# plumk97/pip

Hardware: AMD Instinct MI355X
Metric: GiB/s payload checksummed (device-resident), MTU-9000 TCP batch; Mpkt/s (higher is better)
Workload: dtype u8

## Files before the change

### pip_amd/csrc/pipck_coop.hip

```cpp
#include "pipck_common.hpp"
#include "pipck_device.hpp"

#include <algorithm>

namespace pipck {

constexpr uint32_t kCoopLoadsOnly = 1u << 21;
constexpr uint32_t kCoopNoEnd = 1u << 22;

template <int U>
constexpr int coop_waves_per_simd() { return U >= 32 ? 2 : (U >= 24 ? 3 : (U >= 16 ? 4 : 5)); }

__host__ __device__ constexpr uint32_t coop_pitch(uint32_t k) { return k | 1u; }

template <int U, bool VERIFY, bool NT, bool PROBE>
__device__ __forceinline__ void coop_body(uint32_t* s_part, const uint8_t* __restrict__ arena, uint32_t cpp,
                                          uint32_t len, uint64_t n, uint32_t K, const uint32_t* __restrict__ pseudo,
                                          uint32_t n_flows, const uint32_t* __restrict__ flow_of, uint64_t flow_origin,
                                          uint16_t* __restrict__ out, uint8_t* __restrict__ ok, uint32_t kflags,
                                          uint32_t* __restrict__ err) {
    if (!PROBE) kflags &= ~(kCoopLoadsOnly | kCoopNoEnd);
    const int lane = threadIdx.x & 63;
    const uint32_t w = (uint32_t)__builtin_amdgcn_readfirstlane((int)(threadIdx.x >> 6));
    const uint32_t pitch = coop_pitch(K);
    const uint64_t p0 = (uint64_t)blockIdx.x * K;
    const uint32_t np = (uint32_t)min<uint64_t>((uint64_t)K, n - p0);
    const uint32_t tchunks = np * cpp;
    const uint32_t rows = (tchunks + 63) >> 6;
    const uint32_t nch = (len + 15) >> 4;
    const int tail = nch ? (int)len - 16 * ((int)nch - 1) : 16;
    for (uint32_t i = threadIdx.x; i < 64u * pitch; i += 256) s_part[i] = 0;
    uint32_t Pb = 0;
    bool fbad = false;
    if (pseudo && threadIdx.x < np) {
        const uint64_t pkt = p0 + threadIdx.x;
        Pb = flow_of ? flow_pseudo(pseudo, flow_of[pkt], n_flows, fbad)
                     : pseudo[(uint32_t)((flow_origin + pkt) % n_flows)];
    }
    __syncthreads();
    const buf_t tb = buf_rsrc(reinterpret_cast<const u32x4*>(arena) + p0 * cpp, tchunks * 16u);
    uint32_t* part = s_part + lane * pitch;
    const uint32_t q = 256u / cpp, rm = 256u % cpp;
    uint32_t pkt = (64u * w) / cpp, k0 = (64u * w) % cpp;
    const uint32_t my_rows = rows > w ? (rows - w + 3) >> 2 : 0u;
    u32x4 v[U];
    uint32_t probe = 0;
#pragma unroll
    for (int u = 0; u < U; u++) v[u] = buf_load<NT>(tb, ((w + 4u * u) * 64u + lane) * 16u);
    for (uint32_t j0 = 0; j0 < my_rows; j0 += U) {
#pragma unroll
        for (int u = 0; u < U; u++) {
            const uint32_t j = j0 + u;
            if (j < my_rows && (kflags & kCoopLoadsOnly)) {
                probe += v[u].x;
            } else if (j < my_rows) {
                uint32_t k = k0 + lane, pk = pkt;
                if (k >= cpp) {
                    k -= cpp;
                    pk++;
                }
                u32x4 x = v[u];
                if (k >= nch) x = u32x4{0u, 0u, 0u, 0u};
                else if (k == nch - 1 && tail < 16) x = mask_tail(x, tail);
                if (pk < np) atomicAdd(&part[pk], dot4(x, 0u));
                k0 += rm;
                pkt += q;
                if (k0 >= cpp) {
                    k0 -= cpp;
                    pkt++;
                }
            }
            v[u] = buf_load<NT>(tb, ((w + 4u * (j + U)) * 64u + lane) * 16u);
        }
    }
    __syncthreads();
    if (kflags & (kCoopLoadsOnly | kCoopNoEnd)) {
        if (probe == 0x9E3779B9u) s_part[0] = probe;
        return;
    }
    const uint32_t i = threadIdx.x;
    if (i < np) {
        uint32_t s = 0;
#pragma unroll 16
        for (int l = 0; l < 64; l++) s += s_part[l * pitch + i];
        const uint32_t F = bswap16(fold16(s));
        const uint32_t P = pseudo ? Pb + len_term(len) : 0u;
        if (fbad) flow_refused(err);
        if (VERIFY)
            store_result8(buf_rsrc(ok + p0, np), i, fbad ? 0u : (uint32_t)(fold16(P + F) == 0xFFFFu));
        else
            store_result16(buf_rsrc(out + p0, 2u * np), 2u * i, fbad ? 0u : (uint32_t)finish(P, F));
    }
}

template <int U, bool VERIFY, bool NT>
__global__ __launch_bounds__(256) __attribute__((amdgpu_waves_per_eu(coop_waves_per_simd<U>()))) void k_flat_coop(
    const uint8_t* __restrict__ arena, uint32_t cpp, uint32_t len, uint64_t n, uint32_t K,
    const uint32_t* __restrict__ pseudo, uint32_t n_flows, const uint32_t* __restrict__ flow_of, uint64_t flow_origin,
    uint16_t* __restrict__ out, uint8_t* __restrict__ ok, uint32_t kflags, uint32_t* __restrict__ err) {
    extern __shared__ uint32_t s_part[];
    coop_body<U, VERIFY, NT, false>(s_part, arena, cpp, len, n, K, pseudo, n_flows, flow_of, flow_origin, out, ok,
                                    kflags, err);
}

template <int U, bool VERIFY, bool NT>
__global__ __launch_bounds__(256) __attribute__((amdgpu_waves_per_eu(coop_waves_per_simd<U>()))) void
k_flat_coop_probe(const uint8_t* __restrict__ arena, uint32_t cpp, uint32_t len, uint64_t n, uint32_t K,
                  const uint32_t* __restrict__ pseudo, uint32_t n_flows, const uint32_t* __restrict__ flow_of,
                  uint64_t flow_origin, uint16_t* __restrict__ out, uint8_t* __restrict__ ok, uint32_t kflags,
                  uint32_t* __restrict__ err) {
    extern __shared__ uint32_t s_part[];
    coop_body<U, VERIFY, NT, true>(s_part, arena, cpp, len, n, K, pseudo, n_flows, flow_of, flow_origin, out, ok,
                                   kflags, err);
}

typedef void (*coop_fn)(const uint8_t*, uint32_t, uint32_t, uint64_t, uint32_t, const uint32_t*, uint32_t,
                        const uint32_t*, uint64_t, uint16_t*, uint8_t*, uint32_t, uint32_t*);

int launch_flat_coop(bool verify, const void* d_arena, uint64_t stride, uint32_t len, uint64_t n,
                     const uint32_t* d_pseudo, uint32_t n_flows, const uint32_t* d_flow_of, uint64_t flow_origin,
                     uint16_t* d_out, uint8_t* d_ok, uint32_t* d_err, hipStream_t s, uint32_t rows_per_wave,
                     uint32_t ring, uint32_t kflags) {
    const uint32_t cpp = (uint32_t)(stride / 16);
    const bool jumbo = cpp >= 256;
    const uint32_t rpw = rows_per_wave ? rows_per_wave : (jumbo ? 64u : 48u);
    uint32_t K = (4u * rpw * 64u) / cpp;
    K = std::max<uint32_t>(8u, std::min<uint32_t>(256u, K / 8u * 8u));
    if ((uint64_t)K * cpp * 16u >= (1ull << 31)) return PIPCK_EINVAL;
    const uint64_t blocks = (n + K - 1) / K;
    if (blocks > 0x7FFFFFFFull) return PIPCK_EINVAL;
    const size_t lds = 64u * coop_pitch(K) * sizeof(uint32_t);
    const uint32_t nf = n_flows ? n_flows : 1u;
    const uint32_t u = ring ? ring : 32u;
    static const coop_fn kCoop[3][2] = {
        {k_flat_coop<16, false, true>, k_flat_coop<16, true, true>},
        {k_flat_coop<24, false, true>, k_flat_coop<24, true, true>},
        {k_flat_coop<32, false, true>, k_flat_coop<32, true, true>}};
    static const coop_fn kCoopProbe[3] = {k_flat_coop_probe<16, false, true>, k_flat_coop_probe<24, false, true>,
                                          k_flat_coop_probe<32, false, true>};
    const int ui = u >= 32 ? 2 : (u >= 24 ? 1 : 0);
    const bool probe = (kflags & (kCoopLoadsOnly | kCoopNoEnd)) && !verify;
    PIPCK_LAUNCH(probe ? kCoopProbe[ui] : kCoop[ui][verify], dim3((uint32_t)blocks), dim3(256), lds, s, (const uint8_t*)d_arena, cpp, len, n,
                 K, d_pseudo, nf, d_flow_of, flow_origin, d_out, d_ok, kflags, d_err);
    PIPCK_LAUNCHED("k_flat_coop");
    return PIPCK_OK;
}

}
```

### pip_amd/engine.py

```python
from __future__ import annotations

import ctypes as C

from . import _lib
from ._lib import Desc, Flow4, Flow6, call, check, load

DESC_BYTES = C.sizeof(Desc)


def _torch():
    import torch

    return torch


def _ptr(t) -> C.c_void_p | None:
    return None if t is None else C.c_void_p(t.data_ptr())


def current_stream(device=None) -> C.c_void_p:
    torch = _torch()
    return C.c_void_p(torch.cuda.current_stream(device).cuda_stream)


def require_gpu() -> None:
    torch = _torch()
    if not torch.cuda.is_available():
        raise RuntimeError("pip_amd engine needs a HIP device (gfx950); none is visible")
    load()


_hip = None


def hip_runtime() -> C.CDLL:
    global _hip
    if _hip is None:
        import os

        load()
        paths = set()
        with open("/proc/self/maps") as f:
            for line in f:
                parts = line.split()
                if len(parts) >= 6 and os.path.basename(parts[5]).startswith("libamdhip64.so"):
                    paths.add(os.path.realpath(parts[5]))
        if len(paths) != 1:
            raise RuntimeError(f"expected exactly one HIP runtime mapped in this process, found {sorted(paths)}")
        _hip = C.CDLL(paths.pop(), mode=os.RTLD_NOLOAD | os.RTLD_GLOBAL)
    return _hip


def pci_bus_id(device: int) -> str:
    buf = C.create_string_buffer(64)
    try:
        if hip_runtime().hipDeviceGetPCIBusId(buf, C.c_int(len(buf)), C.c_int(device)) == 0:
            return buf.value.decode()
    except (OSError, RuntimeError):
        pass
    p = _torch().cuda.get_device_properties(device)
    return f"{getattr(p, 'pci_domain_id', 0):04x}:{getattr(p, 'pci_bus_id', 0):02x}:" \
           f"{getattr(p, 'pci_device_id', 0):02x}.0"


def gen_flows(family: int, n_flows: int, seed: int, proto: int, device=None):
    torch = _torch()
    size = C.sizeof(Flow4 if family == 4 else Flow6)
    flows = torch.empty(n_flows * size, dtype=torch.uint8, device=device or "cuda")
    fn = "pipck_gen_flows4" if family == 4 else "pipck_gen_flows6"
    call(fn, _ptr(flows), n_flows, seed, proto, current_stream(flows.device))
    return flows, prepare_flows(family, flows, n_flows)


def prepare_flows(family: int, flows, n_flows: int):
    torch = _torch()
    pseudo = torch.empty(n_flows, dtype=torch.int32, device=flows.device)
    fn = "pipck_flows4_prepare" if family == 4 else "pipck_flows6_prepare"
    call(fn, _ptr(flows), n_flows, _ptr(pseudo), current_stream(flows.device))
    return pseudo


def flows_to_device(family: int, flows_bytes: bytes, device=None):
    torch = _torch()
    t = torch.frombuffer(bytearray(flows_bytes), dtype=torch.uint8).to(device or "cuda")
    return t


def _n_flows(n_flows, pseudo, flow_of) -> int:
    if n_flows is not None:
        return n_flows
    if flow_of is not None and pseudo is not None:
        return pseudo.numel()
    return 1


def checksum_fixed(arena, stride: int, length: int, n: int, pseudo=None, n_flows: int | None = None, flow_of=None,
                   flow_origin: int = 0, out=None, err=None):
    torch = _torch()
    if out is None:
        out = torch.empty(n, dtype=torch.int16, device=arena.device)
    _check_span(arena, stride, length, n)
    call("pipck_checksum_fixed_n", _ptr(arena), stride, length, n, _ptr(pseudo), _n_flows(n_flows, pseudo, flow_of),
         _ptr(flow_of), flow_origin, _ptr(out), _ptr(err), current_stream(arena.device))
    return out


def _bound(fn: str, *args):
    f = getattr(load(), fn)

    def run():
        rc = f(*args)
        if rc:
            check(fn, rc)

    return run


def prepare_checksum_fixed(arena, stride: int, length: int, n: int, pseudo=None, n_flows: int | None = None,
                           flow_of=None, flow_origin: int = 0, out=None, err=None):
    torch = _torch()
    if out is None:
        out = torch.empty(n, dtype=torch.int16, device=arena.device)
    _check_span(arena, stride, length, n)
    return _bound("pipck_checksum_fixed_n", _ptr(arena), stride, length, n, _ptr(pseudo),
                  _n_flows(n_flows, pseudo, flow_of), _ptr(flow_of), flow_origin, _ptr(out), _ptr(err),
                  current_stream(arena.device)), out


def verify_fixed(arena, stride: int, length: int, n: int, pseudo=None, n_flows: int | None = None, flow_of=None,
                 flow_origin: int = 0, ok=None, err=None):
    torch = _torch()
    if ok is None:
        ok = torch.empty(n, dtype=torch.uint8, device=arena.device)
    _check_span(arena, stride, length, n)
    call("pipck_verify_fixed_n", _ptr(arena), stride, length, n, _ptr(pseudo), _n_flows(n_flows, pseudo, flow_of),
         _ptr(flow_of), flow_origin, _ptr(ok), _ptr(err), current_stream(arena.device))
    return ok


def checksum_ragged(arena, desc, pseudo=None, out=None, err=None):
    torch = _torch()
    n = desc.shape[0]
    if out is None:
        out = torch.empty(n, dtype=torch.int16, device=arena.device)
    call("pipck_checksum_ragged_n", _ptr(arena), _nbytes(arena), _ptr(desc), n, _ptr(pseudo),
         pseudo.numel() if pseudo is not None else 0, _ptr(out), _ptr(err), current_stream(arena.device))
    return out


def verify_ragged(arena, desc, pseudo=None, ok=None, err=None):
    torch = _torch()
    n = desc.shape[0]
    if ok is None:
        ok = torch.empty(n, dtype=torch.uint8, device=arena.device)
    call("pipck_verify_ragged_n", _ptr(arena), _nbytes(arena), _ptr(desc), n, _ptr(pseudo),
         pseudo.numel() if pseudo is not None else 0, _ptr(ok), _ptr(err), current_stream(arena.device))
    return ok


def tune_xcd_weights(m=None, period: int = 0) -> None:
    arr = (C.c_uint32 * 8)(*[int(x) for x in m]) if m is not None else None
    call("pipck_tune_xcd_weights", arr, period)


def _nbytes(t) -> int:
    return t.numel() * t.element_size()


def checksum_packed(arena, lens, tile_chunk, n: int | None = None, pseudo=None, n_flows: int | None = None,
                    flow_of=None, flow_origin: int = 0, out=None, err=None):
    torch = _torch()
    n = lens.numel() if n is None else n
    if out is None:
        out = torch.empty(n, dtype=torch.int16, device=arena.device)
    _check_packed(arena, lens, tile_chunk, n)
    call("pipck_checksum_packed_n", _ptr(arena), _nbytes(arena), _ptr(lens), _ptr(tile_chunk), n, _ptr(pseudo),
         _n_flows(n_flows, pseudo, flow_of), _ptr(flow_of), flow_origin, _ptr(out), _ptr(err),
         current_stream(arena.device))
    return out


def verify_packed(arena, lens, tile_chunk, n: int | None = None, pseudo=None, n_flows: int | None = None,
                  flow_of=None, flow_origin: int = 0, ok=None, err=None):
    torch = _torch()
    n = lens.numel() if n is None else n
    if ok is None:
        ok = torch.empty(n, dtype=torch.uint8, device=arena.device)
    _check_packed(arena, lens, tile_chunk, n)
    call("pipck_verify_packed_n", _ptr(arena), _nbytes(arena), _ptr(lens), _ptr(tile_chunk), n, _ptr(pseudo),
         _n_flows(n_flows, pseudo, flow_of), _ptr(flow_of), flow_origin, _ptr(ok), _ptr(err),
         current_stream(arena.device))
    return ok


def packed_index(lens, n: int | None = None):
    torch = _torch()
    n = lens.numel() if n is None else n
    tc = torch.empty((n + 63) // 64 + 1, dtype=torch.int64, device=lens.device)
    call("pipck_packed_index", _ptr(lens), n, _ptr(tc), current_stream(lens.device))
    return tc


_packed_total: dict = {}


def _check_packed(arena, lens, tile_chunk, n, unit: int = 16):
    import weakref

    if n > lens.numel() or tile_chunk.numel() < (n + 63) // 64 + 1:
        raise ValueError("lens / tile_chunk shorter than the batch")
    ent = _packed_total.get(id(tile_chunk))
    if ent is not None and ent[0]() is tile_chunk and ent[1] == tile_chunk._version and ent[2] == n:
        chunks = ent[3]
    else:
        chunks = int(tile_chunk[(n + 63) // 64].item())
        if len(_packed_total) > 64:
            _packed_total.clear()
        _packed_total[id(tile_chunk)] = (weakref.ref(tile_chunk), tile_chunk._version, n, chunks)
    need = unit * chunks if unit == 16 else (chunks + 15) // 16 * 16
    if need > arena.numel() * arena.element_size():
        raise ValueError(f"packed batch needs {need} B, arena has {arena.numel() * arena.element_size()}")


def checksum_packed_bytes(arena, lens, tile_off, n: int | None = None, pseudo=None, n_flows: int | None = None,
                          flow_of=None, flow_origin: int = 0, out=None, err=None):
    torch = _torch()
    n = lens.numel() if n is None else n
    if out is None:
        out = torch.empty(n, dtype=torch.int16, device=arena.device)
    _check_packed(arena, lens, tile_off, n, unit=1)
    call("pipck_checksum_packed_bytes_n", _ptr(arena), _nbytes(arena), _ptr(lens), _ptr(tile_off), n, _ptr(pseudo),
         _n_flows(n_flows, pseudo, flow_of), _ptr(flow_of), flow_origin, _ptr(out), _ptr(err),
         current_stream(arena.device))
    return out


def prepare_checksum_packed_bytes(arena, lens, tile_off, n: int | None = None, pseudo=None,
                                  n_flows: int | None = None, flow_of=None, flow_origin: int = 0, out=None, err=None):
    torch = _torch()
    n = lens.numel() if n is None else n
    if out is None:
        out = torch.empty(n, dtype=torch.int16, device=arena.device)
    _check_packed(arena, lens, tile_off, n, unit=1)
    return _bound("pipck_checksum_packed_bytes_n", _ptr(arena), _nbytes(arena), _ptr(lens), _ptr(tile_off), n,
                  _ptr(pseudo), _n_flows(n_flows, pseudo, flow_of), _ptr(flow_of), flow_origin, _ptr(out),
                  _ptr(err), current_stream(arena.device)), out


def verify_packed_bytes(arena, lens, tile_off, n: int | None = None, pseudo=None, n_flows: int | None = None,
                        flow_of=None, flow_origin: int = 0, ok=None, err=None):
    torch = _torch()
    n = lens.numel() if n is None else n
    if ok is None:
        ok = torch.empty(n, dtype=torch.uint8, device=arena.device)
    _check_packed(arena, lens, tile_off, n, unit=1)
    call("pipck_verify_packed_bytes_n", _ptr(arena), _nbytes(arena), _ptr(lens), _ptr(tile_off), n, _ptr(pseudo),
         _n_flows(n_flows, pseudo, flow_of), _ptr(flow_of), flow_origin, _ptr(ok), _ptr(err),
         current_stream(arena.device))
    return ok


def rx_verify_ring(ring, stride: int, lens, n: int | None = None, ok=None, err=None):
    torch = _torch()
    n = lens.numel() if n is None else n
    if n * stride > _nbytes(ring) or n > lens.numel():
        raise ValueError("ring smaller than n * stride, or fewer lengths than slots")
    if ok is None:
        ok = torch.empty(n, dtype=torch.uint8, device=ring.device)
    call("pipck_rx_verify_ring_n", _ptr(ring), stride, _ptr(lens), n, _ptr(ok), _ptr(err),
         current_stream(ring.device))
    return ok


def rx_verify_device(arena, lens, tile_off, n: int | None = None, ok=None, err=None):
    torch = _torch()
    n = lens.numel() if n is None else n
    if ok is None:
        ok = torch.empty(n, dtype=torch.uint8, device=arena.device)
    _check_packed(arena, lens, tile_off, n, unit=1)
    call("pipck_rx_verify_device", _ptr(arena), _nbytes(arena), _ptr(lens), _ptr(tile_off), n, _ptr(ok), _ptr(err),
         current_stream(arena.device))
    return ok


TX_IP_FILLED, TX_L4_FILLED = 1, 2
TX_UDP_ZERO_AS_ONES = 1


def tx_fill_device(arena, lens, tile_off, n: int | None = None, flags: int = 0, done=None, err=None):
    torch = _torch()
    n = lens.numel() if n is None else n
    if done is None:
        done = torch.empty(n, dtype=torch.uint8, device=arena.device)
    _check_packed(arena, lens, tile_off, n, unit=1)
    call("pipck_tx_fill_device", _ptr(arena), _nbytes(arena), _ptr(lens), _ptr(tile_off), n, flags, _ptr(done),
         _ptr(err), current_stream(arena.device))
    return done


def packed_bytes_index(lens, n: int | None = None):
    torch = _torch()
    n = lens.numel() if n is None else n
    to = torch.empty((n + 63) // 64 + 1, dtype=torch.int64, device=lens.device)
    call("pipck_packed_bytes_index", _ptr(lens), n, _ptr(to), current_stream(lens.device))
    return to


def checksum_chains(arena, segs, seg_begin, pkt_flow=None, pseudo=None, out=None, err=None):
    torch = _torch()
    n_pk = seg_begin.shape[0] - 1
    scratch = torch.empty(max(segs.shape[0], 1), dtype=torch.int32, device=arena.device)
    if out is None:
        out = torch.empty(n_pk, dtype=torch.int16, device=arena.device)
    call("pipck_checksum_chains_n", _ptr(arena), _nbytes(arena), _ptr(segs), segs.shape[0], _ptr(seg_begin),
         _ptr(pkt_flow), n_pk, _ptr(pseudo), pseudo.numel() if pseudo is not None else 0, _ptr(scratch), _ptr(out),
         _ptr(err), current_stream(arena.device))
    return out


def update_fixed(arena, stride: int, n: int, cover_off: int, cover_len: int, ck_off: int, edit_off: int,
                 edit_len: int, new_bytes=None, new_stride: int = 0, pseudo_old=None, pseudo_new=None,
                 n_flows: int | None = None, flow_of=None, flow_origin: int = 0, err=None) -> None:
    if pseudo_old is not None and pseudo_new is not None and pseudo_old.numel() != pseudo_new.numel():
        raise ValueError("pseudo_old and pseudo_new must have the same number of flows")
    _check_span(arena, stride, cover_off + cover_len, n)
    if edit_len and new_bytes is not None and n and \
            (n - 1) * new_stride + edit_len > new_bytes.numel() * new_bytes.element_size():
        raise ValueError("new_bytes is too small for the batch")
    call("pipck_update_fixed_n", _ptr(arena), stride, n, cover_off, cover_len, ck_off, edit_off, edit_len,
         _ptr(new_bytes), new_stride, _ptr(pseudo_old), _ptr(pseudo_new), _n_flows(n_flows, pseudo_old, flow_of),
         _ptr(flow_of), flow_origin, _ptr(err), current_stream(arena.device))


def _check_span(arena, stride, length, n):
    if n and (n - 1) * stride + length > arena.numel() * arena.element_size():
        raise ValueError(f"arena of {arena.numel() * arena.element_size()} B is too small for "
                         f"{n} packets x stride {stride} (len {length})")


def make_desc(offsets, lengths, flows, device=None):
    import numpy as np

    torch = _torch()
    n = len(offsets)
    raw = np.zeros(n, dtype=[("offset", "<u8"), ("len", "<u4"), ("flow", "<u4")])
    raw["offset"], raw["len"], raw["flow"] = offsets, lengths, flows
    return torch.from_numpy(raw.view(np.int64).reshape(n, 2).copy()).to(device or "cuda")


def cfg_seed(cfg: int) -> int:
    return load().pipck_cfg_seed(cfg)


def gen_fixed(arena, stride: int, length: int, n: int, first: int, seed: int, hdr: int) -> None:
    _check_span(arena, stride, length, n)
    if n and (n * stride) > arena.numel() * arena.element_size():
        raise ValueError("arena too small for generated stride slots")
    call("pipck_gen_fixed", _ptr(arena), stride, length, n, first, seed, hdr, current_stream(arena.device))


def gen_ragged(n: int, first: int, seed: int, hdr: int, n_flows: int, device=None, lengths=None):
    torch = _torch()
    dev = device or "cuda"
    if lengths is None:
        lengths = torch.empty(n, dtype=torch.int32, device=dev)
        call("pipck_gen_zipf_lengths", _ptr(lengths), n, first, seed, current_stream(lengths.device))
    desc = torch.empty((n, 2), dtype=torch.int64, device=lengths.device)
    nbytes = C.c_uint64(0)
    call("pipck_gen_ragged_layout", _ptr(lengths), n, first, n_flows, _ptr(desc), C.byref(nbytes),
         current_stream(lengths.device))
    arena = torch.empty(max(int(nbytes.value), 16), dtype=torch.uint8, device=lengths.device)
    call("pipck_gen_ragged_fill", _ptr(arena), _ptr(desc), n, first, seed, hdr, current_stream(arena.device))
    return arena, desc, lengths


def gen_packed(n: int, first: int, seed: int, hdr: int, device=None, lengths=None):
    torch = _torch()
    arena, desc, lengths = gen_ragged(n, first, seed, hdr, 1, device=device, lengths=lengths)
    del desc
    lens16 = lengths.to(torch.int16)
    return arena, lens16, packed_index(lens16, n), lengths


def gen_packed_bytes(n: int, first: int, seed: int, hdr: int, device=None, lengths=None):
    torch = _torch()
    dev = device or "cuda"
    if lengths is None:
        lengths = torch.empty(n, dtype=torch.int32, device=dev)
        call("pipck_gen_zipf_lengths", _ptr(lengths), n, first, seed, current_stream(lengths.device))
    lens16 = lengths.to(torch.int16)
    tile_off = packed_bytes_index(lens16, n)
    total = int(tile_off[(n + 63) // 64].item())
    arena = torch.empty(max((total + 15) // 16 * 16, 16), dtype=torch.uint8, device=lengths.device)
    arena[total:].zero_()
    call("pipck_gen_packed_bytes", _ptr(arena), _ptr(lens16), _ptr(tile_off), n, first, seed, hdr,
         current_stream(arena.device))
    return arena, lens16, tile_off, lengths


def gen_rx_ring(n: int, seed: int, stride: int, l4_len: int = 0):
    torch = _torch()
    arena, lens, _, kind, start, l4 = gen_rx_frames(n, seed, l4_len=l4_len)
    ln = lens.to(torch.int64) & 0xFFFF
    if int(ln.max().item()) > stride:
        raise ValueError("a frame is longer than the slot stride")
    ring = torch.zeros(n * stride, dtype=torch.uint8, device=arena.device)
    step = 1 << 16
    for f0 in range(0, n, step):
        lc, sc = ln[f0:f0 + step], start[f0:f0 + step]
        m = lc.numel()
        frame = torch.repeat_interleave(torch.arange(m, device=arena.device), lc)
        excl = torch.cumsum(lc, 0) - lc
        within = torch.arange(frame.numel(), device=arena.device) - excl[frame]
        ring[(f0 + frame) * stride + within] = arena[sc[frame] + within]
    return ring, lens, kind


def gen_rx_frames(n: int, seed: int, checksummed: bool = True, l4_len: int = 0):
    torch = _torch()
    g = torch.Generator(device="cuda").manual_seed(seed)
    l4 = torch.empty(n, dtype=torch.int32, device="cuda")
    if l4_len:
        l4.fill_(l4_len)
    else:
        call("pipck_gen_zipf_lengths", _ptr(l4), n, 0, cfg_seed(4), current_stream())
    kind = torch.randint(0, 4, (n,), device="cuda", generator=g)
    v6 = kind == 3
    hl = torch.where(v6, 40, 20).to(torch.int64)
    l4 = l4.to(torch.int64)
    frame = l4 + hl
    lens = frame.to(torch.int16)
    tile_off = packed_bytes_index(lens)
    total = int(tile_off[-1].item())
    arena = torch.randint(0, 256, ((total + 16 + 127) // 128 * 128,), dtype=torch.uint8, device="cuda", generator=g)
    start = torch.cumsum(frame, 0) - frame
    proto = torch.where(kind == 2, 17, 6)

    def put(col, val, mask):
        idx = (start + col)[mask]
        arena[idx] = (val[mask] if torch.is_tensor(val) else torch.full_like(idx, val)).to(torch.uint8)

    v4 = ~v6
    put(0, 0x45, v4)
    put(2, frame >> 8, v4)
    put(3, frame & 0xFF, v4)
    put(6, 0, v4)
    put(7, 0, v4)
    put(9, proto, v4)
    put(0, 0x60, v6)
    put(4, l4 >> 8, v6)
    put(5, l4 & 0xFF, v6)
    put(6, 6, v6)
    if not checksummed:
        return arena, lens, tile_off, kind, start, l4
    field = start + hl + torch.where(proto == 6, 16, 6)
    for k in (0, 1):
        arena[field + k] = 0
    put(10, 0, v4)
    put(11, 0, v4)

    def be_words(first, count):
        idx = start[:, None] + first + torch.arange(2 * count, device="cuda")
        b = arena[idx].to(torch.int64)
        return (b[:, 0::2] * 256 + b[:, 1::2]).sum(1)

    pseudo = torch.where(v6, be_words(8, 16), be_words(12, 4)) + proto
    flows = torch.arange(n, device="cuda", dtype=torch.int64)

    def ragged(off, ln, ps):
        desc = torch.stack([off, ln | (flows << 32)], 1)
        return checksum_ragged(arena, desc, ps).to(torch.int64) & 0xFFFF

    r = ragged(start + hl, l4, pseudo.to(torch.int32))
    arena[field] = (r >> 8).to(torch.uint8)
    arena[field + 1] = (r & 0xFF).to(torch.uint8)
    ip = ragged(start, torch.full_like(l4, 20), None)
    put(10, ip >> 8, v4)
    put(11, ip & 0xFF, v4)
    return arena, lens, tile_off, kind, start, l4


def tune(lanes_per_packet: int = 0, loads_per_lane: int = 0, blocks: int = 0, plain_loads: bool = False,
         flat: bool = True, nt_loads: bool = False, rows_per_task: int = 0, xcd_groups: bool = False,
         packed_tiles: bool = True, wide_blocks: bool = False,
         small: bool = True, small_k_log: int = 0, flat_small: bool = True, tiny_tiles: bool = True,
         flat_tiny: bool = True, force_flat_tiny: bool = False, packed_marks_only: bool = False,
         trace: bool = False, loads_only: bool = False, no_task_end: bool = False,
         end_no_store: bool = False, alt_flat_schedule: bool = False,
         plain_result_stores: bool = False, wave_stores: bool = False, free_run: bool = False,
         packed_no_align: bool = False, hdr_in_place: bool = False, ring_own_slots: bool = False,
         ring_all_coop: bool = False, ring_adapt: bool | None = None) -> None:
    if not 0 <= small_k_log <= 4:
        raise ValueError("small_k_log must be 0..4")
    flags = ((1 if plain_loads else 0) | (0 if flat else 2) | (4 if nt_loads else 0) | (8 if xcd_groups else 0)
             | (0 if packed_tiles else 16) | (32 if wide_blocks else 0) | (0 if small else 64)
             | (0 if flat_small else 128) | (rows_per_task << 8) | (0 if tiny_tiles else 1 << 16)
             | (0 if flat_tiny else 1 << 17) | (1 << 18 if force_flat_tiny else 0) | (small_k_log << 24)
             | (1 << 19 if packed_marks_only else 0) | (1 << 20 if trace else 0) | (1 << 21 if loads_only else 0) | (1 << 22 if no_task_end else 0)
             | (1 << 23 if end_no_store else 0) | (1 << 28 if alt_flat_schedule else 0)
             | (1 << 29 if plain_result_stores else 0)
             | (1 << 30 if (wave_stores or packed_no_align) else 0)
             | (1 << 31 if free_run else 0))
    load().pipck_tune(lanes_per_packet, loads_per_lane, blocks, flags)
    load().pipck_tune_probes(1 if hdr_in_place else 0)
    ring = (1 if ring_own_slots else 0) | (2 if ring_all_coop else 0) | {None: 0, False: 4, True: 8}[ring_adapt]
    if ring or hasattr(load(), "pipck_tune_ring"):
        load().pipck_tune_ring(ring)
```

Before: 6740.

## Add fixed-depth jumbo cooperative body, line-aligned task sizing, and relax U32 occupancy

Adds an opt-in jumbo-packet body for the cooperative checksum kernel. When a task's chunks fit in two ring passes, it uses a fully unrolled two-stage load/reduce schedule with branchless tail masking, explicit waitcnt and sched barriers, replacing the generic per-row loop and its bookkeeping. Adds an opt-in task sizing rule that rounds packets-per-block to a cache-line-aligned quantum, and a flag for exact waits. It also raises the occupancy hint for the U=32 kernel from 2 to 3 waves per SIMD, which applies by default and may cause register spills in exchange for more latency hiding.

Result: no change. 6759 (median of 2 runs) (+0.3%).

```diff
diff --git a/pip_amd/csrc/pipck_coop.hip b/pip_amd/csrc/pipck_coop.hip
--- a/pip_amd/csrc/pipck_coop.hip
+++ b/pip_amd/csrc/pipck_coop.hip
@@ -9,7 +9,7 @@
 constexpr uint32_t kCoopNoEnd = 1u << 22;
 
 template <int U>
-constexpr int coop_waves_per_simd() { return U >= 32 ? 2 : (U >= 24 ? 3 : (U >= 16 ? 4 : 5)); }
+constexpr int coop_waves_per_simd() { return U >= 24 ? 3 : (U >= 16 ? 4 : 5); }
 
 __host__ __device__ constexpr uint32_t coop_pitch(uint32_t k) { return k | 1u; }
 
@@ -93,14 +93,117 @@
     }
 }
 
+constexpr uint32_t kCoopLineTasks = 1u << 29;
+constexpr uint32_t kCoopJumboBody = 1u << 30;
+constexpr uint32_t kCoopExactWait = 1u << 31;
+
+__host__ __device__ constexpr bool coop_jumbo_fits(uint32_t cpp, uint32_t K, uint32_t U) {
+    return cpp >= 256u && (uint64_t)K * cpp <= 4ull * 64u * 2u * U;
+}
+
+template <int U, bool NT, bool MASK, bool EXACT>
+__device__ __forceinline__ void coop_rows_jumbo(uint32_t* part, buf_t tb, uint32_t w, int lane, uint32_t cpp,
+                                                uint32_t len, uint32_t np) {
+    asm volatile("; coop_rows_jumbo mask=%0 exact=%1" ::"n"((int)MASK), "n"((int)EXACT) : "memory");
+    const uint32_t nch = (len + 15) >> 4;
+    const Mask128 tm = low_bytes(nch ? (int)len - 16 * ((int)nch - 1) : 0);
+    const uint32_t t0 = (uint32_t)tm.m0, t1 = (uint32_t)(tm.m0 >> 32), t2 = (uint32_t)tm.m1,
+                   t3 = (uint32_t)(tm.m1 >> 32);
+    uint32_t k = 64u * w + (uint32_t)lane, pk = 0;
+    const uint32_t off = k * 16u;
+    auto row = [&](u32x4 x) {
+        uint32_t s;
+        if (MASK) {
+            const bool whole = k + 1u < nch;
+            x.x &= whole ? ~0u : t0;
+            x.y &= whole ? ~0u : t1;
+            x.z &= whole ? ~0u : t2;
+            x.w &= whole ? ~0u : t3;
+            const uint32_t d = dot4(x, 0u);
+            s = k < nch ? d : 0u;
+        } else {
+            s = dot4(x, 0u);
+        }
+        atomicAdd(&part[min(pk, np - 1u)], s);
+        const uint32_t t = k + 256u;
+        pk += t >= cpp ? 1u : 0u;
+        k = min(t, t - cpp);
+        __builtin_amdgcn_sched_barrier(0);
+    };
+    u32x4 v[U];
+#pragma unroll
+    for (int u = 0; u < U; u++) v[u] = buf_load<NT>(tb, off + 4096u * u);
+    if (!EXACT) __builtin_amdgcn_s_waitcnt(0x0F70);
+#pragma unroll
+    for (int u = 0; u < U; u++) {
+        row(v[u]);
+        v[u] = buf_load<NT>(tb, off + 4096u * (U + u));
+    }
+    if (!EXACT) __builtin_amdgcn_s_waitcnt(0x0F70);
+#pragma unroll
+    for (int u = 0; u < U; u++) row(v[u]);
+}
+
+template <int U, bool VERIFY, bool NT>
+__device__ __forceinline__ void coop_body_jumbo(uint32_t* s_part, const uint8_t* __restrict__ arena, uint32_t cpp,
+                                                uint32_t len, uint64_t n, uint32_t K,
+                                                const uint32_t* __restrict__ pseudo, uint32_t n_flows,
+                                                const uint32_t* __restrict__ flow_of, uint64_t flow_origin,
+                                                uint16_t* __restrict__ out, uint8_t* __restrict__ ok, uint32_t kflags,
+                                                uint32_t* __restrict__ err) {
+    const int lane = threadIdx.x & 63;
+    const uint32_t w = (uint32_t)__builtin_amdgcn_readfirstlane((int)(threadIdx.x >> 6));
+    const uint32_t pitch = coop_pitch(K);
+    const uint64_t p0 = (uint64_t)blockIdx.x * K;
+    const uint32_t np = (uint32_t)min<uint64_t>((uint64_t)K, n - p0);
+    const uint32_t tchunks = np * cpp;
+    for (uint32_t i = threadIdx.x; i < 64u * pitch; i += 256) s_part[i] = 0;
+    uint32_t Pb = 0;
+    bool fbad = false;
+    if (pseudo && threadIdx.x < np) {
+        const uint64_t pkt = p0 + threadIdx.x;
+        Pb = flow_of ? flow_pseudo(pseudo, flow_of[pkt], n_flows, fbad)
+                     : pseudo[(uint32_t)((flow_origin + pkt) % n_flows)];
+    }
+    __syncthreads();
+    const buf_t tb = buf_rsrc(reinterpret_cast<const u32x4*>(arena) + p0 * cpp, tchunks * 16u);
+    uint32_t* part = s_part + lane * pitch;
+    const bool exact = (kflags & kCoopExactWait) != 0;
+    if (len == cpp * 16u) {
+        if (exact) coop_rows_jumbo<U, NT, false, true>(part, tb, w, lane, cpp, len, np);
+        else coop_rows_jumbo<U, NT, false, false>(part, tb, w, lane, cpp, len, np);
+    } else {
+        if (exact) coop_rows_jumbo<U, NT, true, true>(part, tb, w, lane, cpp, len, np);
+        else coop_rows_jumbo<U, NT, true, false>(part, tb, w, lane, cpp, len, np);
+    }
+    __syncthreads();
+    const uint32_t i = threadIdx.x;
+    if (i < np) {
+        uint32_t s = 0;
+#pragma unroll 16
+        for (int l = 0; l < 64; l++) s += s_part[l * pitch + i];
+        const uint32_t F = bswap16(fold16(s));
+        const uint32_t P = pseudo ? Pb + len_term(len) : 0u;
+        if (fbad) flow_refused(err);
+        if (VERIFY)
+            store_result8(buf_rsrc(ok + p0, np), i, fbad ? 0u : (uint32_t)(fold16(P + F) == 0xFFFFu));
+        else
+            store_result16(buf_rsrc(out + p0, 2u * np), 2u * i, fbad ? 0u : (uint32_t)finish(P, F));
+    }
+}
+
 template <int U, bool VERIFY, bool NT>
 __global__ __launch_bounds__(256) __attribute__((amdgpu_waves_per_eu(coop_waves_per_simd<U>()))) void k_flat_coop(
     const uint8_t* __restrict__ arena, uint32_t cpp, uint32_t len, uint64_t n, uint32_t K,
     const uint32_t* __restrict__ pseudo, uint32_t n_flows, const uint32_t* __restrict__ flow_of, uint64_t flow_origin,
     uint16_t* __restrict__ out, uint8_t* __restrict__ ok, uint32_t kflags, uint32_t* __restrict__ err) {
     extern __shared__ uint32_t s_part[];
-    coop_body<U, VERIFY, NT, false>(s_part, arena, cpp, len, n, K, pseudo, n_flows, flow_of, flow_origin, out, ok,
-                                    kflags, err);
+    if ((kflags & kCoopJumboBody) && coop_jumbo_fits(cpp, K, U))
+        coop_body_jumbo<U, VERIFY, NT>(s_part, arena, cpp, len, n, K, pseudo, n_flows, flow_of, flow_origin, out, ok,
+                                       kflags, err);
+    else
+        coop_body<U, VERIFY, NT, false>(s_part, arena, cpp, len, n, K, pseudo, n_flows, flow_of, flow_origin, out,
+                                        ok, kflags, err);
 }
 
 template <int U, bool VERIFY, bool NT>
@@ -117,15 +220,28 @@
 typedef void (*coop_fn)(const uint8_t*, uint32_t, uint32_t, uint64_t, uint32_t, const uint32_t*, uint32_t,
                         const uint32_t*, uint64_t, uint16_t*, uint8_t*, uint32_t, uint32_t*);
 
+constexpr uint32_t coop_gcd(uint32_t a, uint32_t b) { return b ? coop_gcd(b, a % b) : a; }
+constexpr uint32_t coop_task_packets(uint64_t stride, uint32_t rows_per_wave, bool line_quantum) {
+    const uint32_t cpp = (uint32_t)(stride / 16);
+    const bool jumbo = cpp >= 256;
+    const uint32_t rpw = rows_per_wave ? rows_per_wave : (jumbo ? 64u : 48u);
+    const uint32_t q = jumbo && line_quantum ? 128u / coop_gcd((uint32_t)(stride % 128u), 128u) : 8u;
+    const uint32_t K = (4u * rpw * 64u) / cpp / q * q;
+    return K < q ? q : (K > 256u ? 256u : K);
+}
+static_assert(coop_task_packets(8992, 0, true) == 28 && coop_task_packets(8960, 0, true) == 29, "cfg5 / cfg3, by line");
+static_assert(coop_task_packets(4096, 0, true) == 64 && coop_task_packets(65536, 0, true) == 4, "jumbo, by line");
+static_assert(coop_task_packets(8992, 54, true) == 24, "rows_per_task = 54: cfg5's default task under the line rule");
+static_assert(coop_task_packets(1488, 0, true) == 128 && coop_task_packets(1488, 0, false) == 128, "cfg2");
+static_assert(coop_task_packets(8992, 0, false) == 24 && coop_task_packets(8960, 0, false) == 24, "cfg5 / cfg3");
+static_assert(coop_task_packets(4096, 0, false) == 64 && coop_task_packets(65536, 0, false) == 8, "jumbo");
+
 int launch_flat_coop(bool verify, const void* d_arena, uint64_t stride, uint32_t len, uint64_t n,
                      const uint32_t* d_pseudo, uint32_t n_flows, const uint32_t* d_flow_of, uint64_t flow_origin,
                      uint16_t* d_out, uint8_t* d_ok, uint32_t* d_err, hipStream_t s, uint32_t rows_per_wave,
                      uint32_t ring, uint32_t kflags) {
     const uint32_t cpp = (uint32_t)(stride / 16);
-    const bool jumbo = cpp >= 256;
-    const uint32_t rpw = rows_per_wave ? rows_per_wave : (jumbo ? 64u : 48u);
-    uint32_t K = (4u * rpw * 64u) / cpp;
-    K = std::max<uint32_t>(8u, std::min<uint32_t>(256u, K / 8u * 8u));
+    const uint32_t K = coop_task_packets(stride, rows_per_wave, (kflags & kCoopLineTasks) != 0);
     if ((uint64_t)K * cpp * 16u >= (1ull << 31)) return PIPCK_EINVAL;
     const uint64_t blocks = (n + K - 1) / K;
     if (blocks > 0x7FFFFFFFull) return PIPCK_EINVAL;
diff --git a/pip_amd/engine.py b/pip_amd/engine.py
--- a/pip_amd/engine.py
+++ b/pip_amd/engine.py
@@ -489,7 +489,9 @@
          end_no_store: bool = False, alt_flat_schedule: bool = False,
          plain_result_stores: bool = False, wave_stores: bool = False, free_run: bool = False,
          packed_no_align: bool = False, hdr_in_place: bool = False, ring_own_slots: bool = False,
-         ring_all_coop: bool = False, ring_adapt: bool | None = None) -> None:
+         ring_all_coop: bool = False, ring_adapt: bool | None = None,
+         coop_jumbo_body: bool = False, coop_exact_wait: bool = False,
+         coop_line_tasks: bool = False) -> None:
     if not 0 <= small_k_log <= 4:
         raise ValueError("small_k_log must be 0..4")
     flags = ((1 if plain_loads else 0) | (0 if flat else 2) | (4 if nt_loads else 0) | (8 if xcd_groups else 0)
@@ -498,9 +500,9 @@
              | (0 if flat_tiny else 1 << 17) | (1 << 18 if force_flat_tiny else 0) | (small_k_log << 24)
              | (1 << 19 if packed_marks_only else 0) | (1 << 20 if trace else 0) | (1 << 21 if loads_only else 0) | (1 << 22 if no_task_end else 0)
              | (1 << 23 if end_no_store else 0) | (1 << 28 if alt_flat_schedule else 0)
-             | (1 << 29 if plain_result_stores else 0)
-             | (1 << 30 if (wave_stores or packed_no_align) else 0)
-             | (1 << 31 if free_run else 0))
+             | (1 << 29 if (plain_result_stores or coop_line_tasks) else 0)
+             | (1 << 30 if (wave_stores or packed_no_align or coop_jumbo_body) else 0)
+             | (1 << 31 if (free_run or coop_exact_wait) else 0))
     load().pipck_tune(lanes_per_packet, loads_per_lane, blocks, flags)
     load().pipck_tune_probes(1 if hdr_in_place else 0)
     ring = (1 if ring_own_slots else 0) | (2 if ring_all_coop else 0) | {None: 0, False: 4, True: 8}[ring_adapt]
```
